# wuliwei9278/primalCR

Measured on AMD Instinct MI355X. Metric: pairwise-comparisons/sec, higher is better.
Workload: dtype f32; 1 GPU; ml1m-shaped PrimalCR++ -k 100 -l 5000 (configs[1]); 6040 users x 3952 items, 939809 ratings, 131347247 ordered pairs; 1 step = 1 outer iteration (V step + U step); solver=PrimalCR++, rank=100, parallelism=user-sharded x1, accumulation=f64, storage=f32

## Files before the change

primalcr_amd/csrc/pcr_host.cpp:

```cpp
#include "pcr_host.h"

#include <algorithm>
#include <atomic>
#include <cerrno>
#include <climits>
#include <cstdint>
#include <cmath>
#include <cstdio>
#include <cstdlib>
#include <cstring>
#include <exception>
#include <functional>
#include <limits>
#include <memory>
#include <mutex>
#include <numeric>
#include <random>
#include <thread>
#include <fcntl.h>
#include <sys/mman.h>
#include <sys/stat.h>
#include <unistd.h>

static thread_local std::string g_err;
// ... 281 lines not shown
        ds->train.item.assign(item, item + nnz);
        ds->train.val.assign(val, val + nnz);
        if (tindex) ds->test.index.assign(tindex, tindex + d1 + 1); else ds->test.index.assign(d1 + 1, 0);
        ds->test.item.assign(titem, titem + tnnz);
        ds->test.val.assign(tval, tval + tnnz);
        ds->tnnz_file = tnnz;
        *out = ds.release();
        return PCR_OK;
    });
}

#include <map>
static std::map<std::string, std::string>& tune_table() { static thread_local std::map<std::string, std::string> t; return t; }
static const char* const TUNE_KEYS[] = {"ustep_mode", "cluster_k", "cluster_users", "ubins", "ustep_gram", "spmm_tiles", "spmm_chunk", "sddmm_csc",
                                        "lanes", "pipeline", "window_cache", "prepare_merged", "resort_window", "allreduce_chunks", "p2p_ll",
                                        "p2p_timeout_ms", "p2p_queue_budget", "count_rows", "debug", "win16", "ustep_win_lds", "plan_key64", "ustep_newton", "vblock_users", "recommend_select", "ranks_batch_users", "sample_threads", "rerank_lds", "ridge_form", "nnls_form", "itemfold_table_bytes", "fault_cluster_member", "fault_p2p_skip", "fault_p2p_coarse", nullptr};
extern "C" int pcr_tune(const char* key, const char* value) {
    if (!key) { pcr_set_error("pcr_tune: null key"); return PCR_ERR_ARG; }
    bool known = false;
    for (const char* const* k = TUNE_KEYS; *k; ++k) known = known || !strcmp(*k, key);
    if (!known) { pcr_set_error(std::string("pcr_tune: unknown key '") + key + "'"); return PCR_ERR_ARG; }
    if (value) tune_table()[key] = value; else tune_table().erase(key);
    return PCR_OK;
}
bool pcr_tune_get(const char* key, std::string* out) {
    auto it = tune_table().find(key);
    if (it == tune_table().end()) return false;
    if (out) *out = it->second;
    return true;
}
int pcr_tune_int(const char* key, int dflt) {
// ... 1731 lines not shown
```

primalcr_amd/csrc/pcr_prims.h:

```cpp
#pragma once
#include <hip/hip_runtime.h>
#include <stdint.h>

#define PCR_WAVE 64

template <typename T> struct VecOf;
template <> struct VecOf<float>  { typedef float4 type;  static constexpr int N = 4; };
template <> struct VecOf<double> { typedef double2 type; static constexpr int N = 2; };

__device__ __forceinline__ float  vdot(const float4& a, const float4& b)  { return a.x * b.x + a.y * b.y + a.z * b.z + a.w * b.w; }
__device__ __forceinline__ double vdot(const double2& a, const double2& b) { return a.x * b.x + a.y * b.y; }
__device__ __forceinline__ float  velem(const float4& a, int e)  { return e == 0 ? a.x : e == 1 ? a.y : e == 2 ? a.z : a.w; }
__device__ __forceinline__ double velem(const double2& a, int e) { return e == 0 ? a.x : a.y; }

struct Geo { int r, ld, nchunk, G; };
__device__ __forceinline__ size_t row_off(int row, const Geo& geo) { return (size_t)((unsigned long long)(unsigned)row * (unsigned)geo.ld); }

template <typename T>
struct Shard {
    int64_t nu, nnz;
    int d2;
    const int64_t* uptr;
    const int32_t* item;
    const uint16_t* lvl;
// ... 288 lines not shown
    const int w[4] = {(int)(wv.x & 0xFFFFu), (int)(wv.x >> 16), (int)(wv.y & 0xFFFFu), (int)(wv.y >> 16)};
    double acc = 0.0;
#pragma unroll
    for (int l = 0; l < 5; ++l) {
        if (l >= nlev || l == lev) continue;
        if (l < lev) {
            const int wi = w[l < 4 ? l : 3], e = rs[l + 1];
            acc += (double)(e - wi) * (xp - shift) - (S[e] - S[wi]);
        } else {
            const int wi = w[l - 1 >= 0 ? l - 1 : 0], s0 = rs[l];
            acc += (double)(wi - s0) * (xp + shift) - (S[wi] - S[s0]);
        }
    }
    return 2.0 * acc;
}
template <typename T, int STRIDE, bool HV, bool WT = false>
__device__ __forceinline__ void sweep_out4(const Shard<T>& S, int64_t s0, int n, int nlev, int tid, const T* xs, const double* Sx,
                                           const int* rs, T* __restrict__ c_out, double cu = 1.0) {
    const uint2* __restrict__ w2 = reinterpret_cast<const uint2*>(reinterpret_cast<const uint16_t*>(S.win) + (size_t)s0 * 4);
    for (int p0 = tid; p0 < n; p0 += STRIDE * 4) {
        uint2 wv[4];
        int lv[4], si[4];
#pragma unroll
        for (int q = 0; q < 4; ++q) {
            const int p = p0 + q * STRIDE;
            if (p < n) { wv[q] = w2[p]; lv[q] = S.slvl[s0 + p]; si[q] = S.sidx[s0 + p]; }
        }
#pragma unroll
        for (int q = 0; q < 4; ++q) {
            const int p = p0 + q * STRIDE;
            if (p < n) {
                const double c = sweep_coeff_win4(wv[q], Sx, rs, nlev, lv[q], (double)xs[p], HV ? 0.0 : 1.0);
                c_out[s0 + si[q]] = (T)(WT ? c * cu : c);
            }
        }
    }
}

template <typename T>
__device__ __forceinline__ double sweep_coeff_cached(const Shard<T>& Sh, size_t row, const double* S, const int* rs, int nlev,
                                                     int lev, double xp, double shift) {
    return Sh.w16 ? sweep_coeff_win(reinterpret_cast<const uint16_t*>(Sh.win) + row * Sh.ws, S, rs, nlev, lev, xp, shift)
                  : sweep_coeff_win(reinterpret_cast<const uint32_t*>(Sh.win) + row * Sh.ws, S, rs, nlev, lev, xp, shift);
}

template <typename T, int BLOCK, class LevF, typename W>
__device__ __forceinline__ double block_objective_win(const T* ms, LevF levf, const int* rs, int nlev, int n,
                                                      const W* __restrict__ win, int ws, double* S, double* red) {
// ... 271 lines not shown
```

primalcr_amd/csrc/pcr_solver.hip:

```cpp
#include <hip/hip_runtime.h>
#include <rccl/rccl.h>

#include <algorithm>
#include <chrono>
#include <cmath>
#include <cstdio>
#include <cstring>
#include <memory>
#include <string>
#include <vector>

#include "pcr_host.h"
#include "pcr_dev.h"
#include "pcr_kernels.h"
#include "pcr_gram.h"
#include "pcr_newton.h"
#include "pcr_vblock.h"
#include "pcr_p2p.h"

#define NCCLCHK(expr)                                                                          \
    do {                                                                                       \
        ncclResult_t e_ = (expr);                                                              \
        if (e_ != ncclSuccess) {                                                               \
            pcr_set_error(std::string(#expr) + ": " + ncclGetErrorString(e_));                 \
            return PCR_ERR_COMM;                                                               \
        }                                                                                      \
    } while (0)
#include "pcr_plan.h"
#include "pcr_plan_dev.h"

#include "pcr_classes.h"

struct Tune {
    int lanes = 0, spmm_chunk = 0, spmm_tiles = 0, sddmm_csc = -1, ustep_mode = 0, cluster_k = 4, cluster_users = 0, window_cache = 1,
        prepare_merged = -1, pipeline = 1, debug = 0, fault_cluster_member = 0, ustep_gram = -1, count_rows = 0, allreduce_chunks = 0,
        resort_window = 8, p2p_ll = 16, p2p_timeout_ms = 20000, p2p_queue_budget = 0, fault_p2p_skip = 0, fault_p2p_coarse = 0, win16 = 1, ustep_win_lds = 1, plan_key64 = 0, ustep_newton = 0, vblock_users = 0, recommend_select = 1;
    std::string ubins;
    void read() {
        lanes = pcr_tune_int("lanes", 0); spmm_chunk = pcr_tune_int("spmm_chunk", 0); spmm_tiles = pcr_tune_int("spmm_tiles", 0);
        sddmm_csc = pcr_tune_int("sddmm_csc", -1); ustep_mode = pcr_tune_int("ustep_mode", 0); cluster_k = pcr_tune_int("cluster_k", 4);
        cluster_users = pcr_tune_int("cluster_users", 0); window_cache = pcr_tune_int("window_cache", 1);
        prepare_merged = pcr_tune_int("prepare_merged", -1);
        pipeline = pcr_tune_int("pipeline", 1); debug = pcr_tune_int("debug", 0); fault_cluster_member = pcr_tune_int("fault_cluster_member", 0);
        ustep_gram = pcr_tune_int("ustep_gram", -1); count_rows = pcr_tune_int("count_rows", 0);
        allreduce_chunks = pcr_tune_int("allreduce_chunks", 0);
        resort_window = pcr_tune_int("resort_window", 8); p2p_ll = pcr_tune_int("p2p_ll", 16);
        p2p_timeout_ms = pcr_tune_int("p2p_timeout_ms", 20000); fault_p2p_skip = pcr_tune_int("fault_p2p_skip", 0);
        fault_p2p_coarse = pcr_tune_int("fault_p2p_coarse", 0); p2p_queue_budget = pcr_tune_int("p2p_queue_budget", 0);
        win16 = pcr_tune_int("win16", 1); ustep_win_lds = pcr_tune_int("ustep_win_lds", 1); plan_key64 = pcr_tune_int("plan_key64", 0); ustep_newton = pcr_tune_int("ustep_newton", 0); vblock_users = pcr_tune_int("vblock_users", 0);
        recommend_select = pcr_tune_int("recommend_select", 1);
        ubins.clear(); pcr_tune_get("ubins", &ubins);
    }
};

template <typename T>
struct Solver final : pcr_solver {
    pcr_params prm;
    Tune tune;
    int rank = 0, nranks = 1;
    int64_t d1 = 0, d2 = 0, tnnz_file = 0;
    Geo geo;
    hipStream_t st = nullptr;
    static constexpr int NSIDE = 12;
    hipStream_t side[NSIDE] = {};
    hipEvent_t ev_fork = nullptr;
// ... 67 lines not shown
        std::vector<double> h_val;
        std::vector<int64_t> h_runofs;
        std::vector<int32_t> h_cnt;
        std::vector<double> h_lgain;
        const uint16_t* elvl_p = nullptr;
        const int64_t* erunofs_p = nullptr;
        const int32_t* erunstart_p = nullptr;
        int idcg_k = -1;
    } ev[2];
    DBuf<double> d_out4;
    std::vector<int32_t> h_test_item;
    std::vector<double> h_test_val;
    DBuf<T> d_U, d_V, d_Vnew, d_g, d_delta, d_rr, d_p, d_Hp;
    CGState* d_cgp = nullptr;
    DBuf<double> d_partA, d_partB, d_scal;
    DBuf<unsigned long long> d_counters;
    DBuf<char> d_scratch;
    size_t scratch_stride = 0;
    int scratch_blocks = 0;
    int u_big_blocks = 0;
    double* h_scal = nullptr;
    double* h_uobj = nullptr;
    bool ustep_pending = false;
    double fin_obj = 0.0;
    int64_t fin_info[2] = {0, 0};
    bool fin_ready = false;
    bool device_join = false;
    CGState* h_cg = nullptr;
    unsigned long long* h_counters = nullptr;
    int ew_blocks = 1, ew_per_block = 1;
// ... 519 lines not shown
            });
            RC(es.gain.upload(gain, st));
        }
        for (auto& bn : es.bins) RC(bn.d_users.upload(bn.users, st));
        return PCR_OK;
    }
    int alloc_factors_and_scratch() {
        const size_t nV = (size_t)d2 * geo.ld, nU = (size_t)n_users * geo.ld;
        RC(d_U.alloc(nU)); RC(d_V.alloc(nV)); RC(d_Vnew.alloc(nV)); RC(d_g.alloc(nV)); RC(d_delta.alloc(nV));
        RC(d_rr.alloc(nV)); RC(d_p.alloc(nV)); RC(d_Hp.alloc(nV));
        HIPCHK(hipMemsetAsync(d_U.p, 0, std::max<size_t>(nU, 1) * sizeof(T), st));
        HIPCHK(hipMemsetAsync(d_V.p, 0, std::max<size_t>(nV, 1) * sizeof(T), st));
        ew_blocks = (int)std::min<int64_t>(1024, std::max<int64_t>(1, cdiv((int64_t)nV, 1024)));
        ew_per_block = cdiv((int64_t)nV, ew_blocks);
        RC(d_partA.alloc(4 * 2048)); RC(d_partB.alloc(4 * 2048)); RC(d_scal.alloc(64));
        RC(d_counters.alloc(4 + 64 + (bar_n + 1) / 2));
        bar_p = reinterpret_cast<unsigned*>(d_counters.p + 4 + 64);
        HIPCHK(hipHostMalloc((void**)&h_scal, 64 * sizeof(double)));
        HIPCHK(hipHostMalloc((void**)&h_uobj, 16 * sizeof(double)));
        static_assert(sizeof(CGState) <= 12 * sizeof(double), "CGState must fit d_scal[32..44)");
        h_cg = reinterpret_cast<CGState*>(h_scal + 32);
        d_cgp = reinterpret_cast<CGState*>(d_scal.p + 32);
        HIPCHK(hipHostMalloc((void**)&h_counters, (4 + 64) * sizeof(unsigned long long)));

        size_t need = 0;
        size_t nbig = 0;
        for (const Bin* b : {&bins[3], &pbins[2]})
            if (!b->users.empty()) { need = std::max(need, prepare_bytes<T>(b->cap, host_pow2(b->cap), b->max_lev + 2, 8)); nbig = std::max(nbig, b->users.size()); }
        for (const Bin* b : {&bins[3], &sbins[2]})
            if (!b->users.empty()) { need = std::max(need, vsweep_bytes<T>(b->cap, b->max_lev + 2, true)); nbig = std::max(nbig, b->users.size()); }
// ... 268 lines not shown
                hipLaunchKernelGGL((k_prepare_all<T, 512>), dim3(nb + cdiv(na, wpb)), dim3(512), lds, st, shp, ba.d_users.p, na, ba.cap, cpa, rsa, wb,
                                   bb.d_users.p, nb, bb.cap, cpb, rsb, nb, d_mcsr.p, strict());
            }
            if (!pbins[2].users.empty()) { ProfScope ps(&prof, pname("prepare", pbins[2]), st, pbins[2].nnz, (int64_t)pbins[2].users.size()); fn(pbins[2], st); }
            HIPCHK(hipGetLastError());
            have_sorted = true;
            sh.prev_valid = 1;
            return PCR_OK;
        }
        RC(for_bins(bins, "prepare", fn));
        have_sorted = true;
        sh.prev_valid = 1;
        return PCR_OK;
    }

    int launch_vsweep(bool hv, const T* A, const int* skip = nullptr) {
        if (hv) { if (sddmm_by_tiles()) RC(launch_sddmm_csc(A, d_b.p, skip)); else RC(launch_sddmm(A, d_sitem.p, d_b.p, skip)); }
        if (hv && vblock_nbp) {
            ProfScope ps(&prof, "vblock_b", st);
            const int64_t tiles = (int64_t)(vblock_nbp / GramMfma<T>::TS) * cdiv(d2, GramMfma<T>::TS);
#ifndef PCR_NO_OPTIONAL_KERNELS
            hipLaunchKernelGGL((k_vblock_b<T>), dim3((unsigned)cdiv(tiles, 4)), dim3(256), 0, st, d_U.p, A, d_blk_user.p, vblock_nbp, d_cpos_dense.p, d2, geo, d_b.p, skip);
#endif
            HIPCHK(hipGetLastError());
        }
        return launch_sweeps(hv, skip, hv && sddmm_by_tiles());
    }
    int launch_sweeps(bool hv, const int* skip, bool b_csr = false) {
        const int bc = (b_csr ? 1 : 0) | (sweep_pf4 ? 2 : 0);
        const bool two = hv && !sh.ws;
        const bool wt = sh.uw != nullptr;
        auto fn = [&](Bin& b, hipStream_t q) {
            const int nus = (int)b.users.size();
            const int rsc = b.max_lev + 2;
            if (b.block == 64) {
                const size_t wb = (vsweep_wave_bytes<T>(b.cap, rsc, two) + 15) & ~(size_t)15;
#define LW(HV, WT) hipLaunchKernelGGL((k_vsweep_wave<T, HV, WT>), dim3(cdiv(nus, 4)), dim3(256), wb * 4, q, sh, b.d_users.p, nus, d_b.p, d_c.p, b.cap, rsc, wb, strict(), skip, bc)
                if (hv) { if (wt) LW(true, true); else LW(true, false); } else { if (wt) LW(false, true); else LW(false, false); }
#undef LW
                return;
            }
            const size_t bigb = vsweep_bytes<T>(b.cap, rsc, two);
            const size_t lds = small_common(b.block) + (b.big ? 0 : bigb);
            const int grid = b.big ? std::min(nus, scratch_blocks) : nus;
#define LV(BL, BG, HV) do { if (wt) LVW(BL, BG, HV, true); else LVW(BL, BG, HV, false); } while (0)
#define LVW(BL, BG, HV, WT) hipLaunchKernelGGL((k_vsweep<T, BL, BG, HV, WT>), dim3(grid), dim3(BL), lds, q, sh, geo, b.d_users.p, nus, d_b.p, d_c.p, b.cap, rsc, d_scratch.p, scratch_stride, strict(), skip, bc)
            if (hv) { if (b.big) LV(512, true, true); else LV(512, false, true); }
            else { if (b.big) LV(512, true, false); else LV(512, false, false); }
#undef LVW
#undef LV
        };
        Bin &ba = sbins[0], &bb = sbins[1];
        if (!ba.users.empty() && !bb.users.empty()) {
            const int na = (int)ba.users.size(), nb = (int)bb.users.size();
            const int rsa = ba.max_lev + 2, rsb = bb.max_lev + 2;
            const size_t wb = (vsweep_wave_bytes<T>(ba.cap, rsa, two) + 15) & ~(size_t)15;
            const int wbs = 512, wpb = wbs / 64;
            const size_t lds = std::max(wb * wpb, small_common(wbs) + vsweep_bytes<T>(bb.cap, rsb, two));
            const int grid = nb + cdiv(na, wpb);
            {
                ProfScope ps(&prof, std::string(hv ? "vhv" : "vgrad") + "/all", st, ba.nnz + bb.nnz, (int64_t)(na + nb));
#define LVA(HV, WBS, MW) do { if (wt) LVAW(HV, WBS, MW, true); else LVAW(HV, WBS, MW, false); } while (0)
#define LVAW(HV, WBS, MW, WT) hipLaunchKernelGGL((k_vsweep_all<T, HV, WBS, MW, WT>), dim3(grid), dim3(WBS), lds, st, sh, ba.d_users.p, na, ba.cap, rsa, wb, \
                                        bb.d_users.p, nb, bb.cap, rsb, nb, d_b.p, d_c.p, strict(), skip, bc)
                const bool dense = lds <= (size_t)40 * 1024;
                if (hv) { if (dense) { LVA(true, 512, 8); } else { LVA(true, 512, 1); } } else { if (dense) { LVA(false, 512, 8); } else { LVA(false, 512, 1); } }
#undef LVAW
#undef LVA
            }
            if (!sbins[2].users.empty()) { ProfScope ps(&prof, pname(hv ? "vhv" : "vgrad", sbins[2]), st, sbins[2].nnz, (int64_t)sbins[2].users.size()); fn(sbins[2], st); }
            HIPCHK(hipGetLastError());
            return PCR_OK;
        }
        RC(for_bins_seq(sbins, hv ? "vhv" : "vgrad", fn));
        return PCR_OK;
    }

    int fin_blocks() const { return (int)std::min<int64_t>(1024, cdiv(d2, 256 / geo.G)); }
    int launch_spmm_range(int r, T* out, const T* base, double beta, const int* skip, const T* dots_rr) {
        if (nnz_local > 0 && rng_blk[r + 1] > rng_blk[r]) {
            ProfScope ps(&prof, "spmm", st);
            hipLaunchKernelGGL((k_spmm<T, 256>), dim3(rng_blk[r + 1] - rng_blk[r]), dim3(256), 0, st, d_c.p, d_c2r.p, d_cuf.p,
                               d_chunk_ptr.p, d_slot_base.p, d_slot_id.p, d_blk_chunks.p + rng_blk[r], d_U.p, d_slab.p, geo, skip);
        }
        const int j0 = (int)rng_item[r], j1 = (int)rng_item[r + 1];
        if (j1 <= j0) return PCR_OK;
        const int grid = n_rng == 1 ? fin_blocks() : (int)std::min<int64_t>(1024, cdiv(j1 - j0, 256 / geo.G));
        ProfScope ps2(&prof, "spmm_fin", st);
        if (dots_rr) hipLaunchKernelGGL((k_spmm_fin<T, 256, true>), dim3(grid), dim3(256), 0, st, d_slab.p, d_item_slot.p, base, beta, j1, out, geo, skip, dots_rr, d_partA.p, j0);
// ... 284 lines not shown
        (void)hipEventDestroy(e0); (void)hipEventDestroy(e1); (void)hipEventDestroy(ef); (void)hipEventDestroy(ej); (void)hipStreamDestroy(sd);
        return PCR_OK;
    }
#endif
    int compute_Ha(const double* a, double* Ha) override {
        RC(need_sorted());
        RC(upload_mat(a, d2, d_p.p));
#ifdef PCR_PIPE_PROBE
        RC(pipe_probe());
        RC(need_sorted());
#endif
        RC(device_hv(d_p.p, d_Hp.p));
        return download_mat(d_Hp.p, d2, Ha);
    }

    int device_cg(int* iters) {
        const int64_t n = (int64_t)d2 * geo.ld;
        {
            ProfScope ps(&prof, "cg", st);
            hipLaunchKernelGGL((k_cg_init<T>), dim3(ew_blocks), dim3(PCR_EW_BLOCK), 0, st, d_g.p, d_delta.p, d_rr.p, d_p.p, n, ew_per_block, d_partA.p);
            hipLaunchKernelGGL(k_cg_init_fin, dim3(1), dim3(PCR_EW_BLOCK), 0, st, d_partA.p, ew_blocks, d_cgp, prm.cg_tol);
        }
        const int* skip = &d_cgp->done;
        const bool fused_dots = single() && n_rng == 1 && !vblock_nbp;
        const bool exact_rr = prm.cg_tol < 1e-5;
        for (int k = 1; k <= prm.cg_max_iter; ++k) {
            RC(device_hv(d_p.p, d_Hp.p, skip, fused_dots ? d_rr.p : nullptr));
            {
                ProfScope ps(&prof, "cg", st);
                if (!fused_dots) hipLaunchKernelGGL((k_cg_a<T>), dim3(ew_blocks), dim3(PCR_EW_BLOCK), 0, st, d_p.p, d_Hp.p, d_rr.p, n, ew_per_block, d_partA.p, d_cgp);
                if (exact_rr) {
                    hipLaunchKernelGGL((k_cg_bc<T, true>), dim3(ew_blocks), dim3(PCR_EW_BLOCK), 0, st, d_p.p, d_Hp.p, d_rr.p, d_delta.p, n, ew_per_block, fused_dots ? fin_blocks() : ew_blocks, d_partA.p, d_cgp, k, d_partB.p);
                    hipLaunchKernelGGL(k_cg_stop, dim3(1), dim3(PCR_EW_BLOCK), 0, st, d_partB.p, ew_blocks, d_cgp, k);
                } else {
                    hipLaunchKernelGGL((k_cg_bc<T, false>), dim3(ew_blocks), dim3(PCR_EW_BLOCK), 0, st, d_p.p, d_Hp.p, d_rr.p, d_delta.p, n, ew_per_block, fused_dots ? fin_blocks() : ew_blocks, d_partA.p, d_cgp, k, (double*)nullptr);
                }
            }
            HIPCHK(hipGetLastError());
        }
        if (iters) {
            HIPCHK(hipMemcpyAsync(h_cg, d_cgp, sizeof(CGState), hipMemcpyDeviceToHost, st));
            RC(sync_checked());
            *iters = h_cg->iters;
        }
        return PCR_OK;
    }
    int solve_delta(const double* g, double* delta, int* iters) override {
        RC(need_sorted());
        RC(upload_mat(g, d2, d_g.p));
        RC(device_cg(iters));
        return download_mat(d_delta.p, d2, delta);
    }

    int update_V(double* now_obj, int* info) override {
        int cg_iters = 0, tries = 0, accepted = 0;
        if (!have_sorted) RC(launch_prepare(d_V.p));
        double prev_obj = 0.0;
        const bool prev_u = !unorm_valid;
        const double unorm2_before = unorm2;
        if (start_sums_queued) start_sums_queued = false;
        else RC(objective_sums(d_objp.p, d_V.p, prev_u, 4));
        RC(device_gradient());
        const bool cg_sync = !prepare_is_single_launch();
        RC(device_cg(cg_sync ? &cg_iters : nullptr));
        double step = prm.stepsize, obj = prev_obj;
        const int64_t n = (int64_t)d2 * geo.ld;
        for (int it = 0; it < 20; ++it) {
            hipLaunchKernelGGL((k_axpy_out<T>), dim3(cdiv(n, 256)), dim3(256), 0, st, d_Vnew.p, d_V.p, d_delta.p, -step, n);
            RC(launch_prepare(d_Vnew.p));
            RC(full_objective(d_Vnew.p, &obj));
            if (!cg_sync) cg_iters = h_cg->iters;
            if (it == 0) prev_obj = h_scal[4] + prm.lambda * ((prev_u ? h_scal[6] : unorm2_before) + h_scal[5]) / 2.0;
            if (ustep_pending) {
                RC(ustep_finish(&fin_obj, fin_info));
                fin_ready = true;
            }
            ++tries;
            if (obj < prev_obj) {
                std::swap(d_V.p, d_Vnew.p);
                accepted = 1;
                break;
            }
            step /= 2.0;
// ... 567 lines not shown
```

primalcr_amd/csrc/pcr_vside.h:

```cpp
#pragma once
#include "pcr_prims.h"

template <typename T, int BLOCK>
__global__ __launch_bounds__(BLOCK) void k_sddmm(const T* __restrict__ U, const T* __restrict__ M,
                                                 const int32_t* __restrict__ ruser, const int32_t* __restrict__ rows,
                                                 int64_t nnz, T* __restrict__ out, Geo geo, int tile, const int* skip,
                                                 const int32_t* __restrict__ perm, const int2* __restrict__ blk_map,
                                                 const int32_t* __restrict__ chunk_ptr) {
    typedef typename VecOf<T>::type V;
    constexpr int VEC = VecOf<T>::N;
    extern __shared__ __attribute__((aligned(16))) char smem[];
    if (skip && *skip) return;
    const int G = geo.G, g = threadIdx.x & (G - 1), grp = threadIdx.x / G, ngrp = BLOCK / G;
    const int span = ngrp * tile;
    int32_t* s_row = reinterpret_cast<int32_t*>(smem);
    int32_t* s_usr = s_row + span;
    int64_t b0 = (int64_t)blockIdx.x * span;
    int nb = (int)((nnz - b0 < span) ? (nnz - b0) : span);
    if (blk_map) {
        const int2 bc = blk_map[blockIdx.x];
        if (bc.y == 0) return;
        b0 = chunk_ptr[bc.x];
        nb = chunk_ptr[bc.x + bc.y] - (int)b0;
    }
// ... 183 lines not shown
    extern __shared__ __attribute__((aligned(16))) char smem[];
    if ((int)blockIdx.x < nblk_b)
        prepare_body<T, WB, false>(smem, S, users_b, nusers_b, m_in, cap_b, cap_pad_b, rs_cap_b, nullptr, 0, strict,
                                   (int)blockIdx.x, nblk_b);
    else
        prepare_body<T, 64, false>(smem + (size_t)(threadIdx.x >> 6) * wave_bytes, S, users_a, nusers_a, m_in, cap_a, cap_pad_a,
                                   rs_cap_a, nullptr, 0, strict, ((int)blockIdx.x - nblk_b) * (WB / 64) + (int)(threadIdx.x >> 6),
                                   ((int)gridDim.x - nblk_b) * (WB / 64));
}

template <typename T>
static inline size_t vsweep_bytes(int cap, int rs_cap, bool two) {
    return carve_bytes(cap, sizeof(T)) * (two ? 2 : 1) + carve_bytes(cap + 1, 8) + carve_bytes(rs_cap, 4);
}

template <typename T, int BLOCK, bool BIG, bool HV, bool WT = false>
__device__ __forceinline__ void vsweep_block_body(char* smem, const Shard<T>& S, const int32_t* __restrict__ users, int nusers,
                                                  const T* __restrict__ bsrc, T* __restrict__ c_out, int cap, int rs_cap,
                                                  char* scratch, size_t stride, int strict, int blk, int nblk, int flags = 0) {
    const int b_csr = flags & 1, pf4 = flags & 2;
    Carver small(smem);
    double* red = small.take<double>(BLOCK / PCR_WAVE + 1);
    Carver big(BIG ? scratch + (size_t)blk * stride : small.p);
    T* ms = big.take<T>(cap);
    T* x = (HV && !S.ws) ? big.take<T>(cap) : ms;
    double* Sx = big.take<double>(cap + 1);
    int* rs = big.take<int>(rs_cap);
    const int tid = threadIdx.x;

    for (int ui = blk; ui < nusers; ui += nblk) {
        const int u = users[ui];
        const int64_t s0 = S.uptr[u];
        const int n = (int)(S.uptr[u + 1] - s0);
        const int nlev = (int)(S.runofs[u + 1] - S.runofs[u]) - 1;
        if (n == 0) continue;
        double cu = 1.0;
        if constexpr (WT) cu = S.uw[u];
        if (!HV || !S.ws) {
#pragma unroll 4
            for (int p = tid; p < n; p += BLOCK) ms[p] = S.ms[s0 + p];
        }
        for (int l = tid; l <= nlev; l += BLOCK) rs[l] = S.runstart[S.runofs[u] + l];
        const T* xs = ms;
        if (HV) {
#pragma unroll 4
            for (int p = tid; p < n; p += BLOCK) x[p] = bsrc[s0 + (b_csr ? S.sidx[s0 + p] : p)];
            xs = x;
        }
        __syncthreads();
        block_excl_scan<BLOCK>([&](int i) { return (double)xs[i]; }, Sx, n, red);
        if (S.ws == 4 && S.w16 && pf4) { sweep_out4<T, BLOCK, HV, WT>(S, s0, n, nlev, tid, xs, Sx, rs, c_out, cu); __syncthreads(); continue; }
        for (int p = tid; p < n; p += BLOCK) {
            const int lev = S.slvl[s0 + p];
            const double c = S.ws
                ? sweep_coeff_cached<T>(S, (size_t)(s0 + p), Sx, rs, nlev, lev, (double)xs[p], HV ? 0.0 : 1.0)
                : sweep_coeff<T>(ms, Sx, rs, nlev, lev, ms[p], (double)xs[p], HV ? 0.0 : 1.0, strict);
            c_out[s0 + S.sidx[s0 + p]] = (T)(WT ? c * cu : c);
        }
        __syncthreads();
    }
}
template <typename T, int BLOCK, bool BIG, bool HV, bool WT = false>
__global__ __launch_bounds__(BLOCK) void k_vsweep(Shard<T> S, Geo geo, const int32_t* __restrict__ users, int nusers,
                                                  const T* __restrict__ bsrc, T* __restrict__ c_out,
                                                  int cap, int rs_cap, char* scratch, size_t stride, int strict, const int* skip,
                                                  int b_csr) {
    extern __shared__ __attribute__((aligned(16))) char smem[];
    if (skip && *skip) return;
    vsweep_block_body<T, BLOCK, BIG, HV, WT>(smem, S, users, nusers, bsrc, c_out, cap, rs_cap, scratch, stride, strict,
                                         (int)blockIdx.x, (int)gridDim.x, b_csr);
}

template <typename T>
static inline size_t vsweep_wave_bytes(int cap, int rs_cap, bool two) {
    return carve_bytes(cap, sizeof(T)) * (two ? 2 : 1) + carve_bytes(cap + 1, 8) + carve_bytes(rs_cap, 4);
}
template <typename T, bool HV, bool WT = false>
__device__ __forceinline__ void vsweep_wave_body(char* smem, const Shard<T>& S, const int32_t* __restrict__ users, int nusers,
                                                 const T* __restrict__ bsrc, T* __restrict__ c_out,
                                                 int cap, int rs_cap, size_t wave_bytes, int strict, int ui, int flags = 0) {
    const int b_csr = flags & 1, pf4 = flags & 2;
    const int lane = threadIdx.x & 63, wid = threadIdx.x >> 6;
    if (ui >= nusers) return;
    Carver big(smem + (size_t)wid * wave_bytes);
    T* ms = big.take<T>(cap);
    T* x = (HV && !S.ws) ? big.take<T>(cap) : ms;
    double* Sx = big.take<double>(cap + 1);
    int* rs = big.take<int>(rs_cap);
    const int u = users[ui];
    const int64_t s0 = S.uptr[u];
    const int n = (int)(S.uptr[u + 1] - s0);
    const int nlev = (int)(S.runofs[u + 1] - S.runofs[u]) - 1;
    if (n == 0) return;
    double cu = 1.0;
    if constexpr (WT) cu = S.uw[u];
    if (!HV || !S.ws) {
#pragma unroll 4
        for (int p = lane; p < n; p += 64) ms[p] = S.ms[s0 + p];
    }
    for (int l = lane; l <= nlev; l += 64) rs[l] = S.runstart[S.runofs[u] + l];
    const T* xs = ms;
    if (HV) {
#pragma unroll 4
        for (int p = lane; p < n; p += 64) x[p] = bsrc[s0 + (b_csr ? S.sidx[s0 + p] : p)];
        xs = x;
    }
    wave_sync();
    double carry = 0.0;
    for (int base = 0; base < n; base += 64) {
        const int i = base + lane;
        const double v = (i < n) ? (double)xs[i] : 0.0;
        const double inc = wave_incl_scan(v);
        if (i < n) Sx[i] = carry + inc - v;
        carry += lane63(inc);
    }
    if (lane == 0) Sx[n] = carry;
    wave_sync();
    if (S.ws == 4 && S.w16 && pf4) { sweep_out4<T, 64, HV, WT>(S, s0, n, nlev, lane, xs, Sx, rs, c_out, cu); return; }
    for (int p = lane; p < n; p += 64) {
        const int lev = S.slvl[s0 + p];
        const double c = S.ws
            ? sweep_coeff_cached<T>(S, (size_t)(s0 + p), Sx, rs, nlev, lev, (double)xs[p], HV ? 0.0 : 1.0)
            : sweep_coeff<T>(ms, Sx, rs, nlev, lev, ms[p], (double)xs[p], HV ? 0.0 : 1.0, strict);
        c_out[s0 + S.sidx[s0 + p]] = (T)(WT ? c * cu : c);
    }
}
template <typename T, bool HV, bool WT = false>
__global__ __launch_bounds__(256) void k_vsweep_wave(Shard<T> S, const int32_t* __restrict__ users, int nusers,
                                                     const T* __restrict__ bsrc, T* __restrict__ c_out,
                                                     int cap, int rs_cap, size_t wave_bytes, int strict, const int* skip, int b_csr) {
    extern __shared__ __attribute__((aligned(16))) char smem[];
    if (skip && *skip) return;
    vsweep_wave_body<T, HV, WT>(smem, S, users, nusers, bsrc, c_out, cap, rs_cap, wave_bytes, strict,
                            (int)blockIdx.x * 4 + (int)(threadIdx.x >> 6), b_csr);
}

template <typename T, bool HV, int WB, int MINW = 1, bool WT = false>
__global__ __launch_bounds__(WB, MINW) void k_vsweep_all(Shard<T> S, const int32_t* __restrict__ users_a, int nusers_a, int cap_a,
                                                    int rs_cap_a, size_t wave_bytes, const int32_t* __restrict__ users_b,
                                                    int nusers_b, int cap_b, int rs_cap_b, int nblk_b,
                                                    const T* __restrict__ bsrc, T* __restrict__ c_out, int strict, const int* skip, int b_csr) {
    extern __shared__ __attribute__((aligned(16))) char smem[];
    if (skip && *skip) return;
    if ((int)blockIdx.x < nblk_b)
        vsweep_block_body<T, WB, false, HV, WT>(smem, S, users_b, nusers_b, bsrc, c_out, cap_b, rs_cap_b, nullptr, 0, strict,
                                            (int)blockIdx.x, nblk_b, b_csr);
    else
        vsweep_wave_body<T, HV, WT>(smem, S, users_a, nusers_a, bsrc, c_out, cap_a, rs_cap_a, wave_bytes, strict,
                                ((int)blockIdx.x - nblk_b) * (WB / 64) + (int)(threadIdx.x >> 6), b_csr);
}

template <typename T, int BLOCK>
__global__ __launch_bounds__(BLOCK) void k_spmm(const T* __restrict__ c, const int32_t* __restrict__ c2r,
                                                const int32_t* __restrict__ cuf,
                                                const int32_t* __restrict__ chunk_ptr, const int32_t* __restrict__ inc_base,
                                                const int32_t* __restrict__ slot_id, const int2* __restrict__ blk_chunks,
                                                const T* __restrict__ U, T* __restrict__ slab, Geo geo, const int* skip) {
    typedef typename VecOf<T>::type V;
    constexpr int VEC = VecOf<T>::N;
    if (skip && *skip) return;
    const int G = geo.G, g = threadIdx.x & (G - 1);
    const int2 bc = blk_chunks[blockIdx.x];
    if ((int)threadIdx.x / G >= bc.y) return;
    const int gid = bc.x + (int)threadIdx.x / G;
// ... 219 lines not shown
    for (int64_t i = lo + threadIdx.x; i < hi; i += PCR_EW_BLOCK) {
        const double pv = (double)p[i], h = (double)Hp[i], r = (double)rr[i];
        x += pv * h; y += r * pv; z += r * h; w += h * h;
    }
    x = block_sum<PCR_EW_BLOCK>(x, red);
    y = block_sum<PCR_EW_BLOCK>(y, red);
    z = block_sum<PCR_EW_BLOCK>(z, red);
    w = block_sum<PCR_EW_BLOCK>(w, red);
    if (threadIdx.x == 0) { part[4 * blockIdx.x] = x; part[4 * blockIdx.x + 1] = y; part[4 * blockIdx.x + 2] = z; part[4 * blockIdx.x + 3] = w; }
}

template <typename T, bool EXACT>
__global__ __launch_bounds__(PCR_EW_BLOCK) void k_cg_bc(T* __restrict__ p, const T* __restrict__ Hp, T* __restrict__ rr,
                                                         T* __restrict__ delta, int64_t n, int per_block, int nblk,
                                                         const double* __restrict__ part, CGState* st, int k,
                                                         double* __restrict__ part_rr) {
    __shared__ double red[PCR_EW_BLOCK / PCR_WAVE + 1];
    const int da = st->done_at;
    if (da != 0 && da < k) return;
    double s4[4];
    for (int c = 0; c < 4; ++c) {
        double x = 0.0;
        for (int i = threadIdx.x; i < nblk; i += PCR_EW_BLOCK) x += part[4 * i + c];
        s4[c] = block_sum<PCR_EW_BLOCK>(x, red);
    }
    const double pHp = s4[0], rp = s4[1], rHp0 = s4[2], HpHp = s4[3];
    const double rr2_old = st->rr2buf[(k - 1) & 1];
    const double alpha = -1.0 * rp / pHp;
    double rr2 = rr2_old + 2.0 * alpha * rHp0 + alpha * alpha * HpHp;
    rr2 = rr2 > 0.0 ? rr2 : 0.0;
    const double rHp = rHp0 + alpha * HpHp;
    const bool conv = !EXACT && sqrt(rr2) < st->err;
    const double beta = rHp / pHp;
    const int64_t lo = (int64_t)blockIdx.x * per_block;
    const int64_t hi = (lo + per_block < n) ? lo + per_block : n;
    double x2 = 0.0;
    for (int64_t i = lo + threadIdx.x; i < hi; i += PCR_EW_BLOCK) {
        const double pv = (double)p[i], hv = (double)Hp[i];
        delta[i] = (T)((double)delta[i] + pv * alpha);
        const T rn = (T)((double)rr[i] + hv * alpha);
        rr[i] = rn;
        if (EXACT) x2 += (double)rn * (double)rn;
        if (!conv) p[i] = (T)((double)rn * -1.0 + pv * beta);
    }
    if (EXACT) {
        x2 = block_sum<PCR_EW_BLOCK>(x2, red);
        if (threadIdx.x == 0) { part_rr[2 * blockIdx.x] = x2; part_rr[2 * blockIdx.x + 1] = 0.0; }
    }
    if (blockIdx.x == gridDim.x - 1 && threadIdx.x == 0) {
        st->pHp = pHp; st->rp = rp; st->alpha = alpha; st->rr2 = rr2; st->rHp = rHp; st->beta = beta;
        st->iters += 1;
        if (!EXACT) {
            st->rr2buf[k & 1] = rr2;
            if (conv) { st->done_at = k; st->done = 1; }
        }
    }
}
__global__ __launch_bounds__(PCR_EW_BLOCK) void k_cg_stop(const double* __restrict__ part_rr, int nblk, CGState* st, int k) {
    __shared__ double red[PCR_EW_BLOCK / PCR_WAVE + 1];
    if (st->done) return;
    double a, b;
    reduce_partials2(part_rr, nblk, &a, &b, red);
    if (threadIdx.x == 0) {
        st->rr2 = a; st->rr2buf[k & 1] = a;
        if (sqrt(a) < st->err) { st->done_at = k; st->done = 1; }
    }
}
```

Before: 48.11 billion pairs/s.

## Skip the final CG Hessian SpMM by computing pHp from sweep coefficients

On the last CG iteration, single-rank runs skip the full Hessian-vector product and its SpMM. The value p'Hp is instead rebuilt as lambda*p'p plus a sum of x*c accumulated inside the V-sweep kernels, with p'p and r'p gathered by the previous k_cg_bc. A new k_cg_last kernel applies the delta update and also writes Vnew = V - step*delta, so the first line-search axpy is skipped. This adds new kernel variants and an extra partial-sum buffer, and it risks small numeric differences in pHp from the changed summation order.

```diff
diff --git a/primalcr_amd/csrc/pcr_host.cpp b/primalcr_amd/csrc/pcr_host.cpp
--- a/primalcr_amd/csrc/pcr_host.cpp
+++ b/primalcr_amd/csrc/pcr_host.cpp
@@ -319,7 +319,7 @@
 static std::map<std::string, std::string>& tune_table() { static thread_local std::map<std::string, std::string> t; return t; }
 static const char* const TUNE_KEYS[] = {"ustep_mode", "cluster_k", "cluster_users", "ubins", "ustep_gram", "spmm_tiles", "spmm_chunk", "sddmm_csc",
                                         "lanes", "pipeline", "window_cache", "prepare_merged", "resort_window", "allreduce_chunks", "p2p_ll",
-                                        "p2p_timeout_ms", "p2p_queue_budget", "count_rows", "debug", "win16", "ustep_win_lds", "plan_key64", "ustep_newton", "vblock_users", "recommend_select", "ranks_batch_users", "sample_threads", "rerank_lds", "ridge_form", "nnls_form", "itemfold_table_bytes", "fault_cluster_member", "fault_p2p_skip", "fault_p2p_coarse", nullptr};
+                                        "p2p_timeout_ms", "p2p_queue_budget", "count_rows", "debug", "win16", "ustep_win_lds", "plan_key64", "ustep_newton", "vblock_users", "recommend_select", "cg_last_spmm", "ranks_batch_users", "sample_threads", "rerank_lds", "ridge_form", "nnls_form", "itemfold_table_bytes", "fault_cluster_member", "fault_p2p_skip", "fault_p2p_coarse", nullptr};
 extern "C" int pcr_tune(const char* key, const char* value) {
     if (!key) { pcr_set_error("pcr_tune: null key"); return PCR_ERR_ARG; }
     bool known = false;
diff --git a/primalcr_amd/csrc/pcr_prims.h b/primalcr_amd/csrc/pcr_prims.h
--- a/primalcr_amd/csrc/pcr_prims.h
+++ b/primalcr_amd/csrc/pcr_prims.h
@@ -326,9 +326,9 @@
     }
     return 2.0 * acc;
 }
-template <typename T, int STRIDE, bool HV, bool WT = false>
+template <typename T, int STRIDE, bool HV, bool WT = false, bool BC = false>
 __device__ __forceinline__ void sweep_out4(const Shard<T>& S, int64_t s0, int n, int nlev, int tid, const T* xs, const double* Sx,
-                                           const int* rs, T* __restrict__ c_out, double cu = 1.0) {
+                                           const int* rs, T* __restrict__ c_out, double cu = 1.0, double* bc = nullptr) {
     const uint2* __restrict__ w2 = reinterpret_cast<const uint2*>(reinterpret_cast<const uint16_t*>(S.win) + (size_t)s0 * 4);
     for (int p0 = tid; p0 < n; p0 += STRIDE * 4) {
         uint2 wv[4];
@@ -343,7 +343,9 @@
             const int p = p0 + q * STRIDE;
             if (p < n) {
                 const double c = sweep_coeff_win4(wv[q], Sx, rs, nlev, lv[q], (double)xs[p], HV ? 0.0 : 1.0);
-                c_out[s0 + si[q]] = (T)(WT ? c * cu : c);
+                const T ct = (T)(WT ? c * cu : c);
+                c_out[s0 + si[q]] = ct;
+                if constexpr (BC) *bc += (double)xs[p] * (double)ct;
             }
         }
     }
diff --git a/primalcr_amd/csrc/pcr_solver.hip b/primalcr_amd/csrc/pcr_solver.hip
--- a/primalcr_amd/csrc/pcr_solver.hip
+++ b/primalcr_amd/csrc/pcr_solver.hip
@@ -34,7 +34,7 @@
 struct Tune {
     int lanes = 0, spmm_chunk = 0, spmm_tiles = 0, sddmm_csc = -1, ustep_mode = 0, cluster_k = 4, cluster_users = 0, window_cache = 1,
         prepare_merged = -1, pipeline = 1, debug = 0, fault_cluster_member = 0, ustep_gram = -1, count_rows = 0, allreduce_chunks = 0,
-        resort_window = 8, p2p_ll = 16, p2p_timeout_ms = 20000, p2p_queue_budget = 0, fault_p2p_skip = 0, fault_p2p_coarse = 0, win16 = 1, ustep_win_lds = 1, plan_key64 = 0, ustep_newton = 0, vblock_users = 0, recommend_select = 1;
+        resort_window = 8, p2p_ll = 16, p2p_timeout_ms = 20000, p2p_queue_budget = 0, fault_p2p_skip = 0, fault_p2p_coarse = 0, win16 = 1, ustep_win_lds = 1, plan_key64 = 0, ustep_newton = 0, vblock_users = 0, recommend_select = 1, cg_last_spmm = 0;
     std::string ubins;
     void read() {
         lanes = pcr_tune_int("lanes", 0); spmm_chunk = pcr_tune_int("spmm_chunk", 0); spmm_tiles = pcr_tune_int("spmm_tiles", 0);
@@ -48,7 +48,7 @@
         p2p_timeout_ms = pcr_tune_int("p2p_timeout_ms", 20000); fault_p2p_skip = pcr_tune_int("fault_p2p_skip", 0);
         fault_p2p_coarse = pcr_tune_int("fault_p2p_coarse", 0); p2p_queue_budget = pcr_tune_int("p2p_queue_budget", 0);
         win16 = pcr_tune_int("win16", 1); ustep_win_lds = pcr_tune_int("ustep_win_lds", 1); plan_key64 = pcr_tune_int("plan_key64", 0); ustep_newton = pcr_tune_int("ustep_newton", 0); vblock_users = pcr_tune_int("vblock_users", 0);
-        recommend_select = pcr_tune_int("recommend_select", 1);
+        recommend_select = pcr_tune_int("recommend_select", 1); cg_last_spmm = pcr_tune_int("cg_last_spmm", 0);
         ubins.clear(); pcr_tune_get("ubins", &ubins);
     }
 };
@@ -146,6 +146,7 @@
     DBuf<T> d_U, d_V, d_Vnew, d_g, d_delta, d_rr, d_p, d_Hp;
     CGState* d_cgp = nullptr;
     DBuf<double> d_partA, d_partB, d_scal;
+    DBuf<double> d_partBC, d_partPR;
     DBuf<unsigned long long> d_counters;
     DBuf<char> d_scratch;
     size_t scratch_stride = 0;
@@ -695,6 +696,11 @@
         ew_blocks = (int)std::min<int64_t>(1024, std::max<int64_t>(1, cdiv((int64_t)nV, 1024)));
         ew_per_block = cdiv((int64_t)nV, ew_blocks);
         RC(d_partA.alloc(4 * 2048)); RC(d_partB.alloc(4 * 2048)); RC(d_scal.alloc(64));
+        {
+            size_t nsw = 1;
+            for (auto& b : sbins) nsw += b.users.size();
+            RC(d_partBC.alloc(nsw)); RC(d_partPR.alloc(2 * 1024));
+        }
         RC(d_counters.alloc(4 + 64 + (bar_n + 1) / 2));
         bar_p = reinterpret_cast<unsigned*>(d_counters.p + 4 + 64);
         HIPCHK(hipHostMalloc((void**)&h_scal, 64 * sizeof(double)));
@@ -993,7 +999,7 @@
         return PCR_OK;
     }
 
-    int launch_vsweep(bool hv, const T* A, const int* skip = nullptr) {
+    int launch_vsweep(bool hv, const T* A, const int* skip = nullptr, int* nbc = nullptr) {
         if (hv) { if (sddmm_by_tiles()) RC(launch_sddmm_csc(A, d_b.p, skip)); else RC(launch_sddmm(A, d_sitem.p, d_b.p, skip)); }
         if (hv && vblock_nbp) {
             ProfScope ps(&prof, "vblock_b", st);
@@ -1003,10 +1009,12 @@
 #endif
             HIPCHK(hipGetLastError());
         }
-        return launch_sweeps(hv, skip, hv && sddmm_by_tiles());
-    }
-    int launch_sweeps(bool hv, const int* skip, bool b_csr = false) {
+        return launch_sweeps(hv, skip, hv && sddmm_by_tiles(), nbc);
+    }
+    int launch_sweeps(bool hv, const int* skip, bool b_csr = false, int* nbc = nullptr) {
         const int bc = (b_csr ? 1 : 0) | (sweep_pf4 ? 2 : 0);
+        const bool emit = hv && nbc;
+        int bc_at = 0;
         const bool two = hv && !sh.ws;
         const bool wt = sh.uw != nullptr;
         auto fn = [&](Bin& b, hipStream_t q) {
@@ -1015,7 +1023,10 @@
             if (b.block == 64) {
                 const size_t wb = (vsweep_wave_bytes<T>(b.cap, rsc, two) + 15) & ~(size_t)15;
 #define LW(HV, WT) hipLaunchKernelGGL((k_vsweep_wave<T, HV, WT>), dim3(cdiv(nus, 4)), dim3(256), wb * 4, q, sh, b.d_users.p, nus, d_b.p, d_c.p, b.cap, rsc, wb, strict(), skip, bc)
-                if (hv) { if (wt) LW(true, true); else LW(true, false); } else { if (wt) LW(false, true); else LW(false, false); }
+#define LWB(WT) hipLaunchKernelGGL((k_vsweep_wave_bc<T, WT>), dim3(cdiv(nus, 4)), dim3(256), wb * 4, q, sh, b.d_users.p, nus, d_b.p, d_c.p, b.cap, rsc, wb, strict(), skip, bc, d_partBC.p + bc_at)
+                if (emit) { if (wt) LWB(true); else LWB(false); bc_at += cdiv(nus, 4); }
+                else if (hv) { if (wt) LW(true, true); else LW(true, false); } else { if (wt) LW(false, true); else LW(false, false); }
+#undef LWB
 #undef LW
                 return;
             }
@@ -1024,8 +1035,14 @@
             const int grid = b.big ? std::min(nus, scratch_blocks) : nus;
 #define LV(BL, BG, HV) do { if (wt) LVW(BL, BG, HV, true); else LVW(BL, BG, HV, false); } while (0)
 #define LVW(BL, BG, HV, WT) hipLaunchKernelGGL((k_vsweep<T, BL, BG, HV, WT>), dim3(grid), dim3(BL), lds, q, sh, geo, b.d_users.p, nus, d_b.p, d_c.p, b.cap, rsc, d_scratch.p, scratch_stride, strict(), skip, bc)
-            if (hv) { if (b.big) LV(512, true, true); else LV(512, false, true); }
+#define LVB(BG, WT) hipLaunchKernelGGL((k_vsweep_bc<T, 512, BG, WT>), dim3(grid), dim3(512), lds, q, sh, geo, b.d_users.p, nus, d_b.p, d_c.p, b.cap, rsc, d_scratch.p, scratch_stride, strict(), skip, bc, d_partBC.p + bc_at)
+            if (emit) {
+                if (b.big) { if (wt) LVB(true, true); else LVB(true, false); } else { if (wt) LVB(false, true); else LVB(false, false); }
+                bc_at += grid;
+            }
+            else if (hv) { if (b.big) LV(512, true, true); else LV(512, false, true); }
             else { if (b.big) LV(512, true, false); else LV(512, false, false); }
+#undef LVB
 #undef LVW
 #undef LV
         };
@@ -1043,15 +1060,24 @@
 #define LVAW(HV, WBS, MW, WT) hipLaunchKernelGGL((k_vsweep_all<T, HV, WBS, MW, WT>), dim3(grid), dim3(WBS), lds, st, sh, ba.d_users.p, na, ba.cap, rsa, wb, \
                                         bb.d_users.p, nb, bb.cap, rsb, nb, d_b.p, d_c.p, strict(), skip, bc)
                 const bool dense = lds <= (size_t)40 * 1024;
-                if (hv) { if (dense) { LVA(true, 512, 8); } else { LVA(true, 512, 1); } } else { if (dense) { LVA(false, 512, 8); } else { LVA(false, 512, 1); } }
+#define LVAB(MW, WT) hipLaunchKernelGGL((k_vsweep_all_bc<T, 512, MW, WT>), dim3(grid), dim3(512), lds, st, sh, ba.d_users.p, na, ba.cap, rsa, wb, \
+                                        bb.d_users.p, nb, bb.cap, rsb, nb, d_b.p, d_c.p, strict(), skip, bc, d_partBC.p + bc_at)
+                if (emit) {
+                    if (dense) { if (wt) LVAB(6, true); else LVAB(6, false); } else { if (wt) LVAB(1, true); else LVAB(1, false); }
+                    bc_at += grid;
+                }
+                else if (hv) { if (dense) { LVA(true, 512, 8); } else { LVA(true, 512, 1); } } else { if (dense) { LVA(false, 512, 8); } else { LVA(false, 512, 1); } }
+#undef LVAB
 #undef LVAW
 #undef LVA
             }
             if (!sbins[2].users.empty()) { ProfScope ps(&prof, pname(hv ? "vhv" : "vgrad", sbins[2]), st, sbins[2].nnz, (int64_t)sbins[2].users.size()); fn(sbins[2], st); }
             HIPCHK(hipGetLastError());
+            if (emit) *nbc = bc_at;
             return PCR_OK;
         }
         RC(for_bins_seq(sbins, hv ? "vhv" : "vgrad", fn));
+        if (emit) *nbc = bc_at;
         return PCR_OK;
     }
 
@@ -1366,7 +1392,7 @@
         return download_mat(d_Hp.p, d2, Ha);
     }
 
-    int device_cg(int* iters) {
+    int device_cg(int* iters, T* Vnew = nullptr, double step = 0.0, bool* wrote_vnew = nullptr) {
         const int64_t n = (int64_t)d2 * geo.ld;
         {
             ProfScope ps(&prof, "cg", st);
@@ -1376,16 +1402,28 @@
         const int* skip = &d_cgp->done;
         const bool fused_dots = single() && n_rng == 1 && !vblock_nbp;
         const bool exact_rr = prm.cg_tol < 1e-5;
+        const bool short_last = (nranks == 1 || local_only) && n_rng == 1 && !vblock_nbp && prm.cg_max_iter >= 2 && !tune.cg_last_spmm;
+        if (wrote_vnew) *wrote_vnew = short_last && Vnew;
         for (int k = 1; k <= prm.cg_max_iter; ++k) {
+            if (short_last && k == prm.cg_max_iter) {
+                int nbc = 0;
+                RC(launch_vsweep(true, d_p.p, skip, &nbc));
+                ProfScope ps(&prof, "cg", st);
+                hipLaunchKernelGGL((k_cg_last<T>), dim3(ew_blocks), dim3(PCR_EW_BLOCK), 0, st, d_p.p, d_delta.p, n, ew_per_block, d_partPR.p, ew_blocks, d_partBC.p, nbc,
+                                   rank == 0 ? prm.lambda : 0.0, d_cgp, k, d_V.p, Vnew, -step);
+                HIPCHK(hipGetLastError());
+                break;
+            }
+            double* part_last = short_last && k == prm.cg_max_iter - 1 ? d_partPR.p : nullptr;
             RC(device_hv(d_p.p, d_Hp.p, skip, fused_dots ? d_rr.p : nullptr));
             {
                 ProfScope ps(&prof, "cg", st);
                 if (!fused_dots) hipLaunchKernelGGL((k_cg_a<T>), dim3(ew_blocks), dim3(PCR_EW_BLOCK), 0, st, d_p.p, d_Hp.p, d_rr.p, n, ew_per_block, d_partA.p, d_cgp);
                 if (exact_rr) {
-                    hipLaunchKernelGGL((k_cg_bc<T, true>), dim3(ew_blocks), dim3(PCR_EW_BLOCK), 0, st, d_p.p, d_Hp.p, d_rr.p, d_delta.p, n, ew_per_block, fused_dots ? fin_blocks() : ew_blocks, d_partA.p, d_cgp, k, d_partB.p);
+                    hipLaunchKernelGGL((k_cg_bc<T, true>), dim3(ew_blocks), dim3(PCR_EW_BLOCK), 0, st, d_p.p, d_Hp.p, d_rr.p, d_delta.p, n, ew_per_block, fused_dots ? fin_blocks() : ew_blocks, d_partA.p, d_cgp, k, d_partB.p, part_last);
                     hipLaunchKernelGGL(k_cg_stop, dim3(1), dim3(PCR_EW_BLOCK), 0, st, d_partB.p, ew_blocks, d_cgp, k);
                 } else {
-                    hipLaunchKernelGGL((k_cg_bc<T, false>), dim3(ew_blocks), dim3(PCR_EW_BLOCK), 0, st, d_p.p, d_Hp.p, d_rr.p, d_delta.p, n, ew_per_block, fused_dots ? fin_blocks() : ew_blocks, d_partA.p, d_cgp, k, (double*)nullptr);
+                    hipLaunchKernelGGL((k_cg_bc<T, false>), dim3(ew_blocks), dim3(PCR_EW_BLOCK), 0, st, d_p.p, d_Hp.p, d_rr.p, d_delta.p, n, ew_per_block, fused_dots ? fin_blocks() : ew_blocks, d_partA.p, d_cgp, k, (double*)nullptr, part_last);
                 }
             }
             HIPCHK(hipGetLastError());
@@ -1414,11 +1452,12 @@
         else RC(objective_sums(d_objp.p, d_V.p, prev_u, 4));
         RC(device_gradient());
         const bool cg_sync = !prepare_is_single_launch();
-        RC(device_cg(cg_sync ? &cg_iters : nullptr));
         double step = prm.stepsize, obj = prev_obj;
+        bool have_vnew = false;
+        RC(device_cg(cg_sync ? &cg_iters : nullptr, d_Vnew.p, step, &have_vnew));
         const int64_t n = (int64_t)d2 * geo.ld;
         for (int it = 0; it < 20; ++it) {
-            hipLaunchKernelGGL((k_axpy_out<T>), dim3(cdiv(n, 256)), dim3(256), 0, st, d_Vnew.p, d_V.p, d_delta.p, -step, n);
+            if (it > 0 || !have_vnew) hipLaunchKernelGGL((k_axpy_out<T>), dim3(cdiv(n, 256)), dim3(256), 0, st, d_Vnew.p, d_V.p, d_delta.p, -step, n);
             RC(launch_prepare(d_Vnew.p));
             RC(full_objective(d_Vnew.p, &obj));
             if (!cg_sync) cg_iters = h_cg->iters;
diff --git a/primalcr_amd/csrc/pcr_vside.h b/primalcr_amd/csrc/pcr_vside.h
--- a/primalcr_amd/csrc/pcr_vside.h
+++ b/primalcr_amd/csrc/pcr_vside.h
@@ -221,8 +221,8 @@
     return carve_bytes(cap, sizeof(T)) * (two ? 2 : 1) + carve_bytes(cap + 1, 8) + carve_bytes(rs_cap, 4);
 }
 
-template <typename T, int BLOCK, bool BIG, bool HV, bool WT = false>
-__device__ __forceinline__ void vsweep_block_body(char* smem, const Shard<T>& S, const int32_t* __restrict__ users, int nusers,
+template <typename T, int BLOCK, bool BIG, bool HV, bool WT = false, bool BC = false>
+__device__ __forceinline__ double vsweep_block_body(char* smem, const Shard<T>& S, const int32_t* __restrict__ users, int nusers,
                                                   const T* __restrict__ bsrc, T* __restrict__ c_out, int cap, int rs_cap,
                                                   char* scratch, size_t stride, int strict, int blk, int nblk, int flags = 0) {
     const int b_csr = flags & 1, pf4 = flags & 2;
@@ -234,6 +234,7 @@
     double* Sx = big.take<double>(cap + 1);
     int* rs = big.take<int>(rs_cap);
     const int tid = threadIdx.x;
+    double bc = 0.0;
 
     for (int ui = blk; ui < nusers; ui += nblk) {
         const int u = users[ui];
@@ -256,16 +257,19 @@
         }
         __syncthreads();
         block_excl_scan<BLOCK>([&](int i) { return (double)xs[i]; }, Sx, n, red);
-        if (S.ws == 4 && S.w16 && pf4) { sweep_out4<T, BLOCK, HV, WT>(S, s0, n, nlev, tid, xs, Sx, rs, c_out, cu); __syncthreads(); continue; }
+        if (S.ws == 4 && S.w16 && pf4) { sweep_out4<T, BLOCK, HV, WT, BC>(S, s0, n, nlev, tid, xs, Sx, rs, c_out, cu, &bc); __syncthreads(); continue; }
         for (int p = tid; p < n; p += BLOCK) {
             const int lev = S.slvl[s0 + p];
             const double c = S.ws
                 ? sweep_coeff_cached<T>(S, (size_t)(s0 + p), Sx, rs, nlev, lev, (double)xs[p], HV ? 0.0 : 1.0)
                 : sweep_coeff<T>(ms, Sx, rs, nlev, lev, ms[p], (double)xs[p], HV ? 0.0 : 1.0, strict);
-            c_out[s0 + S.sidx[s0 + p]] = (T)(WT ? c * cu : c);
+            const T ct = (T)(WT ? c * cu : c);
+            c_out[s0 + S.sidx[s0 + p]] = ct;
+            if constexpr (BC) bc += (double)xs[p] * (double)ct;
         }
         __syncthreads();
     }
+    return bc;
 }
 template <typename T, int BLOCK, bool BIG, bool HV, bool WT = false>
 __global__ __launch_bounds__(BLOCK) void k_vsweep(Shard<T> S, Geo geo, const int32_t* __restrict__ users, int nusers,
@@ -282,13 +286,13 @@
 static inline size_t vsweep_wave_bytes(int cap, int rs_cap, bool two) {
     return carve_bytes(cap, sizeof(T)) * (two ? 2 : 1) + carve_bytes(cap + 1, 8) + carve_bytes(rs_cap, 4);
 }
-template <typename T, bool HV, bool WT = false>
-__device__ __forceinline__ void vsweep_wave_body(char* smem, const Shard<T>& S, const int32_t* __restrict__ users, int nusers,
+template <typename T, bool HV, bool WT = false, bool BC = false>
+__device__ __forceinline__ double vsweep_wave_body(char* smem, const Shard<T>& S, const int32_t* __restrict__ users, int nusers,
                                                  const T* __restrict__ bsrc, T* __restrict__ c_out,
                                                  int cap, int rs_cap, size_t wave_bytes, int strict, int ui, int flags = 0) {
     const int b_csr = flags & 1, pf4 = flags & 2;
     const int lane = threadIdx.x & 63, wid = threadIdx.x >> 6;
-    if (ui >= nusers) return;
+    if (ui >= nusers) return 0.0;
     Carver big(smem + (size_t)wid * wave_bytes);
     T* ms = big.take<T>(cap);
     T* x = (HV && !S.ws) ? big.take<T>(cap) : ms;
@@ -298,7 +302,8 @@
     const int64_t s0 = S.uptr[u];
     const int n = (int)(S.uptr[u + 1] - s0);
     const int nlev = (int)(S.runofs[u + 1] - S.runofs[u]) - 1;
-    if (n == 0) return;
+    if (n == 0) return 0.0;
+    double bc = 0.0;
     double cu = 1.0;
     if constexpr (WT) cu = S.uw[u];
     if (!HV || !S.ws) {
@@ -323,14 +328,17 @@
     }
     if (lane == 0) Sx[n] = carry;
     wave_sync();
-    if (S.ws == 4 && S.w16 && pf4) { sweep_out4<T, 64, HV, WT>(S, s0, n, nlev, lane, xs, Sx, rs, c_out, cu); return; }
+    if (S.ws == 4 && S.w16 && pf4) { sweep_out4<T, 64, HV, WT, BC>(S, s0, n, nlev, lane, xs, Sx, rs, c_out, cu, &bc); return bc; }
     for (int p = lane; p < n; p += 64) {
         const int lev = S.slvl[s0 + p];
         const double c = S.ws
             ? sweep_coeff_cached<T>(S, (size_t)(s0 + p), Sx, rs, nlev, lev, (double)xs[p], HV ? 0.0 : 1.0)
             : sweep_coeff<T>(ms, Sx, rs, nlev, lev, ms[p], (double)xs[p], HV ? 0.0 : 1.0, strict);
-        c_out[s0 + S.sidx[s0 + p]] = (T)(WT ? c * cu : c);
-    }
+        const T ct = (T)(WT ? c * cu : c);
+        c_out[s0 + S.sidx[s0 + p]] = ct;
+        if constexpr (BC) bc += (double)xs[p] * (double)ct;
+    }
+    return bc;
 }
 template <typename T, bool HV, bool WT = false>
 __global__ __launch_bounds__(256) void k_vsweep_wave(Shard<T> S, const int32_t* __restrict__ users, int nusers,
@@ -355,6 +363,51 @@
     else
         vsweep_wave_body<T, HV, WT>(smem, S, users_a, nusers_a, bsrc, c_out, cap_a, rs_cap_a, wave_bytes, strict,
                                 ((int)blockIdx.x - nblk_b) * (WB / 64) + (int)(threadIdx.x >> 6), b_csr);
+}
+
+template <int BLOCK>
+__device__ __forceinline__ void store_bc(double bc, char* smem, double* __restrict__ part_bc) {
+    const double t = block_sum<BLOCK>(bc, reinterpret_cast<double*>(smem));
+    if (threadIdx.x == 0) part_bc[blockIdx.x] = t;
+}
+template <typename T, int BLOCK, bool BIG, bool WT>
+__global__ __launch_bounds__(BLOCK) void k_vsweep_bc(Shard<T> S, Geo geo, const int32_t* __restrict__ users, int nusers,
+                                                     const T* __restrict__ bsrc, T* __restrict__ c_out,
+                                                     int cap, int rs_cap, char* scratch, size_t stride, int strict, const int* skip,
+                                                     int b_csr, double* __restrict__ part_bc) {
+    extern __shared__ __attribute__((aligned(16))) char smem[];
+    if (skip && *skip) return;
+    const double bc = vsweep_block_body<T, BLOCK, BIG, true, WT, true>(smem, S, users, nusers, bsrc, c_out, cap, rs_cap, scratch, stride,
+                                                                        strict, (int)blockIdx.x, (int)gridDim.x, b_csr);
+    store_bc<BLOCK>(bc, smem, part_bc);
+}
+template <typename T, bool WT>
+__global__ __launch_bounds__(256) void k_vsweep_wave_bc(Shard<T> S, const int32_t* __restrict__ users, int nusers,
+                                                        const T* __restrict__ bsrc, T* __restrict__ c_out,
+                                                        int cap, int rs_cap, size_t wave_bytes, int strict, const int* skip, int b_csr,
+                                                        double* __restrict__ part_bc) {
+    extern __shared__ __attribute__((aligned(16))) char smem[];
+    if (skip && *skip) return;
+    const double bc = vsweep_wave_body<T, true, WT, true>(smem, S, users, nusers, bsrc, c_out, cap, rs_cap, wave_bytes, strict,
+                                                          (int)blockIdx.x * 4 + (int)(threadIdx.x >> 6), b_csr);
+    store_bc<256>(bc, smem, part_bc);
+}
+template <typename T, int WB, int MINW, bool WT>
+__global__ __launch_bounds__(WB, MINW) void k_vsweep_all_bc(Shard<T> S, const int32_t* __restrict__ users_a, int nusers_a, int cap_a,
+                                                       int rs_cap_a, size_t wave_bytes, const int32_t* __restrict__ users_b,
+                                                       int nusers_b, int cap_b, int rs_cap_b, int nblk_b,
+                                                       const T* __restrict__ bsrc, T* __restrict__ c_out, int strict, const int* skip, int b_csr,
+                                                       double* __restrict__ part_bc) {
+    extern __shared__ __attribute__((aligned(16))) char smem[];
+    if (skip && *skip) return;
+    double bc;
+    if ((int)blockIdx.x < nblk_b)
+        bc = vsweep_block_body<T, WB, false, true, WT, true>(smem, S, users_b, nusers_b, bsrc, c_out, cap_b, rs_cap_b, nullptr, 0, strict,
+                                                             (int)blockIdx.x, nblk_b, b_csr);
+    else
+        bc = vsweep_wave_body<T, true, WT, true>(smem, S, users_a, nusers_a, bsrc, c_out, cap_a, rs_cap_a, wave_bytes, strict,
+                                                 ((int)blockIdx.x - nblk_b) * (WB / 64) + (int)(threadIdx.x >> 6), b_csr);
+    store_bc<WB>(bc, smem, part_bc);
 }
 
 template <typename T, int BLOCK>
@@ -604,7 +657,7 @@
 __global__ __launch_bounds__(PCR_EW_BLOCK) void k_cg_bc(T* __restrict__ p, const T* __restrict__ Hp, T* __restrict__ rr,
                                                          T* __restrict__ delta, int64_t n, int per_block, int nblk,
                                                          const double* __restrict__ part, CGState* st, int k,
-                                                         double* __restrict__ part_rr) {
+                                                         double* __restrict__ part_rr, double* __restrict__ part_last) {
     __shared__ double red[PCR_EW_BLOCK / PCR_WAVE + 1];
     const int da = st->done_at;
     if (da != 0 && da < k) return;
@@ -624,18 +677,27 @@
     const double beta = rHp / pHp;
     const int64_t lo = (int64_t)blockIdx.x * per_block;
     const int64_t hi = (lo + per_block < n) ? lo + per_block : n;
-    double x2 = 0.0;
+    double x2 = 0.0, pp = 0.0, rp1 = 0.0;
     for (int64_t i = lo + threadIdx.x; i < hi; i += PCR_EW_BLOCK) {
         const double pv = (double)p[i], hv = (double)Hp[i];
         delta[i] = (T)((double)delta[i] + pv * alpha);
         const T rn = (T)((double)rr[i] + hv * alpha);
         rr[i] = rn;
         if (EXACT) x2 += (double)rn * (double)rn;
-        if (!conv) p[i] = (T)((double)rn * -1.0 + pv * beta);
+        if (!conv) {
+            const T pn = (T)((double)rn * -1.0 + pv * beta);
+            p[i] = pn;
+            if (part_last) { pp += (double)pn * (double)pn; rp1 += (double)rn * (double)pn; }
+        }
     }
     if (EXACT) {
         x2 = block_sum<PCR_EW_BLOCK>(x2, red);
         if (threadIdx.x == 0) { part_rr[2 * blockIdx.x] = x2; part_rr[2 * blockIdx.x + 1] = 0.0; }
+    }
+    if (part_last) {
+        pp = block_sum<PCR_EW_BLOCK>(pp, red);
+        rp1 = block_sum<PCR_EW_BLOCK>(rp1, red);
+        if (threadIdx.x == 0) { part_last[2 * blockIdx.x] = pp; part_last[2 * blockIdx.x + 1] = rp1; }
     }
     if (blockIdx.x == gridDim.x - 1 && threadIdx.x == 0) {
         st->pHp = pHp; st->rp = rp; st->alpha = alpha; st->rr2 = rr2; st->rHp = rHp; st->beta = beta;
@@ -646,6 +708,36 @@
         }
     }
 }
+template <typename T>
+__global__ __launch_bounds__(PCR_EW_BLOCK) void k_cg_last(const T* __restrict__ p, T* __restrict__ delta, int64_t n, int per_block,
+                                                           const double* __restrict__ part_pr, int nblk_pr,
+                                                           const double* __restrict__ part_bc, int nbc, double lambda, CGState* st, int k,
+                                                           const T* __restrict__ V, T* __restrict__ Vnew, double s) {
+    __shared__ double red[PCR_EW_BLOCK / PCR_WAVE + 1];
+    const int da = st->done_at;
+    const bool idle = da != 0 && da < k;
+    if (idle && !Vnew) return;
+    double pHp = 0.0, rp = 0.0, alpha = 0.0;
+    if (!idle) {
+        double pp, bc = 0.0;
+        reduce_partials2(part_pr, nblk_pr, &pp, &rp, red);
+        for (int i = threadIdx.x; i < nbc; i += PCR_EW_BLOCK) bc += part_bc[i];
+        bc = block_sum<PCR_EW_BLOCK>(bc, red);
+        pHp = lambda * pp + bc;
+        alpha = -1.0 * rp / pHp;
+    }
+    const int64_t lo = (int64_t)blockIdx.x * per_block;
+    const int64_t hi = (lo + per_block < n) ? lo + per_block : n;
+    for (int64_t i = lo + threadIdx.x; i < hi; i += PCR_EW_BLOCK) {
+        T d = delta[i];
+        if (!idle) { d = (T)((double)d + (double)p[i] * alpha); delta[i] = d; }
+        if (Vnew) Vnew[i] = (T)((double)V[i] + s * (double)d);
+    }
+    if (!idle && blockIdx.x == gridDim.x - 1 && threadIdx.x == 0) {
+        st->pHp = pHp; st->rp = rp; st->alpha = alpha;
+        st->iters += 1;
+    }
+}
 __global__ __launch_bounds__(PCR_EW_BLOCK) void k_cg_stop(const double* __restrict__ part_rr, int nblk, CGState* st, int k) {
     __shared__ double red[PCR_EW_BLOCK / PCR_WAVE + 1];
     if (st->done) return;
```

Result: slower. 46.48 billion pairs/s (-3.4%).
